# manyeyes/AliParaformerAsr

Hardware: AMD Instinct MI355X
Metric: RTFx (audio-sec/wall-sec), paraformer-large offline, batch 32x30s per GPU, 2 batches in flight per GPU (higher is better)
Workload: dtype f16; 1 GPU; paraformer-large-zh offline, batch 32x30 s synthetic 16 kHz per GPU (BASELINE.json configs[1]), seeded synthetic weights; global_batch=32, samples_per_utt=480000, T_lfr=500, L=167, steps_in_flight=2

## Files before the change

aliparaformerasr_amd/_native.py:

```python
from __future__ import annotations

import ctypes as C
import os

_HERE = os.path.dirname(os.path.abspath(__file__))
LIB_PATH = os.path.join(_HERE, "libparaformer_hip.so")

PF_OK = 0
PF_ERR_INVALID_ARG = -1
PF_ERR_DEVICE = -2
PF_ERR_IO = -3
PF_ERR_FORMAT = -4
PF_ERR_CAPACITY = -5
PF_ERR_UNSUPPORTED = -6
PF_ERR_DISPOSED = -7
PF_ERR_TOKENS = -8
PF_ERR_NULL_SAMPLES = -9
PF_ERR_RECOGNITION = -10

PF_DECODE_SCORES = 1
PF_DECODE_CTC = 2
PF_DECODE_TOPK = 8
PF_DECODE_CTC_BEAM = 16
PF_HOTWORD_STATES_MAX = 4096
# ... 220 lines not shown
    "pf_host_group_sim": (C.c_int, [C.c_int32, C.c_int32, _i32, C.c_int32, C.c_int32, C.c_int32, C.c_int32, C.c_int32, _i64,
                                    C.c_int32, _i32, _i32]),
    "pf_profile_enable": (C.c_int, [_vp, C.c_int32]),
    "pf_profile_reset": (C.c_int, [_vp]),
    "pf_profile_select": (C.c_int, [_vp, C.c_char_p]),
    "pf_profile_get": (C.c_int, [_vp, C.c_char_p, _P(C.c_double), _i64, _P(C.c_double)]),
    "pf_profile_kernel": (C.c_int, [_vp, C.c_char_p, C.c_char_p, C.c_int32]),
    "pf_last_flops": (C.c_int, [_vp, _P(C.c_double)]),
    "pf_op_lfr_cmvn_pad": (C.c_int, [_vp, _P(_f), _i32, C.c_int32, C.c_int32, _f, C.c_int64, _i32]),
    "pf_op_fbank_batch": (C.c_int, [_vp, _P(_f), _i64, C.c_int32, _f, C.c_int64, _i32]),
    "pf_op_qlinear": (C.c_int, [_vp, _f, _f, _f, C.c_int32, C.c_int32, C.c_int32, C.c_int32, C.c_int32, _f, _P(C.c_uint8), _f,
                                _P(C.c_uint8), _f, _i32]),
    "pf_op_argmax": (C.c_int, [_vp, _f, C.c_int64, C.c_int32, _i64]),
    "pf_op_gemm": (C.c_int, [_vp, _f, _f, _f, C.c_int32, C.c_int32, C.c_int32, C.c_int32, _f]),
    "pf_op_gemm_ex": (C.c_int, [_vp, _P(PfGemmDesc), _f, _f, _f]),
    "pf_op_gemm_rc": (C.c_int, [_vp, _P(PfGemmRcDesc), _f, _f, _f, _f, _f]),
    "pf_op_ffn": (C.c_int, [_vp, _f, _f, _f, _f, _f, _f, C.c_int32, C.c_int32, C.c_int32, _f]),
    "pf_op_ffn_fused": (C.c_int, [_vp, _f, _f, _f, _f, _f, _f, _f, _f, C.c_int32, _f, _f]),
    "pf_op_dec_ffn_fused": (C.c_int, [_vp, C.c_void_p, _f, _f, _f]),
    "pf_op_attn_ffn_fused": (C.c_int, [_vp, _vp, _f, _f]),
    "pf_op_fsmn_enc": (C.c_int, [_vp, _f, _f, C.c_int32, C.c_int32, C.c_int32, C.c_int32, _f]),
    "pf_op_linear32": (C.c_int, [_vp, _f, _f, _f, _f, C.c_int32, C.c_int32, C.c_int32, C.c_int32, _f]),
    "pf_op_ffn32": (C.c_int, [_vp, _f, _f, _f, _f, _f, C.c_int32, C.c_int32, C.c_int32, _f]),
    "pf_op_fsmn_dec": (C.c_int, [_vp, _f, _f, _i32, C.c_int32, C.c_int32, C.c_int32, C.c_int32, _f]),
    "pf_op_lstm": (C.c_int, [_vp, _f, _f, C.c_int32, C.c_int32, C.c_int32, C.c_int32, C.c_int32, _f]),
    "pf_op_us_peak": (C.c_int, [_vp, _f, _f, _f, C.c_float, C.c_float, _i32, C.c_float, C.c_int32, C.c_int32, C.c_int32, _f, _f, _f]),
    "pf_op_logsoftmax_argmax": (C.c_int, [_vp, _f, C.c_int64, C.c_int32, _f, _i64]),
    "pf_op_layernorm": (C.c_int, [_vp, _f, _f, _f, C.c_int64, C.c_int32, _f]),
    "pf_op_attention": (C.c_int, [_vp, _f, _f, _f, C.c_int32, C.c_int32, C.c_int32, C.c_int32, _f]),
    "pf_op_fsmn": (C.c_int, [_vp, _f, _f, _f, C.c_int32, C.c_int32, C.c_int32, C.c_int32, _f]),
# ... 115 lines not shown
```

aliparaformerasr_amd/csrc/c_api.cpp:

```cpp
#include <algorithm>
#include <cstring>
#include <deque>
#include <memory>
#include <mutex>

#include "engine.h"
#include "group.h"
#include "online.h"
#include "recognizer.h"
#include "shards_sim.h"

namespace pf {
static thread_local std::string g_last_error;
void set_last_error(const std::string& m) { g_last_error = m; }
}

using namespace pf;

struct pf_engine {
  std::mutex mu;
  std::shared_ptr<Engine> e;
};
struct pf_recognizer {
  std::mutex mu;
// ... 1003 lines not shown
  e->op_qlinear(x, W, bias, M, N, K, relu, x_is_f16, y, xq_out, aparams_out, wq_out, wscale_out, wzp_out);
  return PF_OK;
  PF_CATCH
}
int pf_op_gemm_ex(pf_engine* h, const pf_gemm_desc* d, const float* A, const float* W, float* C) {
  PF_TRY
  std::shared_ptr<Engine> eh_ = E(h);
  Engine* e = eh_.get();
  NEED(d); NEED(A); NEED(W); NEED(C);
  PF_CHECK(d->struct_size == (int32_t)sizeof(pf_gemm_desc), PF_ERR_INVALID_ARG, "pf_gemm_desc.struct_size mismatch");
  std::lock_guard<std::mutex> lk(e->mutex());
  e->op_gemm_ex(*d, A, W, C);
  return PF_OK;
  PF_CATCH
}
int pf_op_gemm_rc(pf_engine* h, const pf_gemm_rc_desc* d, const float* A, const float* W, float* x_out, float* n16_out,
                  float* n32_out) {
  PF_TRY
  std::shared_ptr<Engine> eh_ = E(h);
  Engine* e = eh_.get();
  NEED(d); NEED(A); NEED(W);
  PF_CHECK(d->struct_size == (int32_t)sizeof(pf_gemm_rc_desc), PF_ERR_INVALID_ARG, "pf_gemm_rc_desc.struct_size mismatch");
  PF_CHECK(x_out || n16_out || n32_out, PF_ERR_INVALID_ARG, "gemm_rc: no output requested");
  std::lock_guard<std::mutex> lk(e->mutex());
  e->op_gemm_rc(*d, A, W, x_out, n16_out, n32_out);
  return PF_OK;
  PF_CATCH
}
int pf_op_ffn(pf_engine* h, const float* x, const float* w1, const float* b1, const float* w2, const float* b2,
              const float* resid, int32_t M, int32_t D, int32_t F, float* y) {
// ... 1131 lines not shown
```

aliparaformerasr_amd/csrc/engine.cpp:

```cpp
#include "engine.h"

#include <algorithm>
#include <cmath>
#include <cstdlib>
#include <chrono>
#include <cstring>
#include <set>

#include "hostutil.h"

namespace pf {

static std::mutex g_main_mu;
static std::vector<std::pair<int, hipStream_t>> g_main_streams;
static std::vector<hipStream_t> g_parked;

Engine::Engine(const pf_engine_config& cfg) {
  device_ = cfg.device;
  int ndev = 0;
  hipError_t e = hipGetDeviceCount(&ndev);
  if (e != hipSuccess || ndev <= 0)
    throw Error(PF_ERR_DEVICE, "no HIP device available (this library has no CPU fallback)");
  PF_CHECK(device_ >= 0 && device_ < ndev, PF_ERR_DEVICE, "device ordinal out of range");
  PF_HIP(hipSetDevice(device_));
// ... 12 lines not shown
  fc_.dither_seed = (uint32_t)cfg.dither_seed;
  fc_.window = cfg.window ? cfg.window : "hamming";
  PF_CHECK(fc_.dither >= 0.f && fc_.dither == fc_.dither, PF_ERR_INVALID_ARG, "dither must be >= 0");
  PF_CHECK(fc_.fs == 16000, PF_ERR_UNSUPPORTED, "only fs = 16000 is supported");
  PF_CHECK((cfg.frame_length_ms == 0 || cfg.frame_length_ms == 25) && (cfg.frame_shift_ms == 0 || cfg.frame_shift_ms == 10),
           PF_ERR_UNSUPPORTED, "only frame_length = 25 ms and frame_shift = 10 ms are supported");
  PF_CHECK(cfg.math_mode >= 0 && cfg.math_mode <= 3, PF_ERR_INVALID_ARG,
           "math_mode must be 0 (f16 MFMA), 1 (fp32 MFMA), 2 (dynamic int8 as model.int8.onnx, int8 MFMA) or 3 (exact: split-f16 products)");
  fp32_mode_ = cfg.math_mode == 1 || cfg.math_mode == 3;
  x3_mode_ = cfg.math_mode == 3;
  int8_mode_ = cfg.math_mode == 2;
  { const char* e = getenv("PF_QKV_MIN"); if (e && e[0]) qkv_split_min_tiles_ = atoi(e); }
  { const char* e = getenv("PF_QKV_FILL"); if (e && e[0]) qkv_split_min_fill_ = atoi(e); }
  { const char* e = getenv("PF_FFN_MIN"); if (e && e[0]) ffn_fused_min_rows_ = atoi(e); }
  { const char* e = getenv("PF_DEC_MID"); if (e && e[0]) dec_mid_ = e[0] != '0'; }

  std::vector<float> shift, scale;
  if (cfg.mvn_path && cfg.mvn_path[0]) {
    parse_mvn_text(read_text_file(cfg.mvn_path), shift, scale);
  } else if (cfg.cmvn_shift && cfg.cmvn_scale && cfg.cmvn_dim > 0) {
    shift.assign(cfg.cmvn_shift, cfg.cmvn_shift + cfg.cmvn_dim);
    scale.assign(cfg.cmvn_scale, cfg.cmvn_scale + cfg.cmvn_dim);
  }
  if (!shift.empty()) {
    PF_CHECK(shift.size() == scale.size(), PF_ERR_FORMAT, "am.mvn: shift/scale length mismatch");
    PF_CHECK((int)shift.size() == fc_.lfr_m * fc_.n_mels, PF_ERR_FORMAT, "am.mvn: CMVN dim must equal lfr_m * n_mels");
  }

  uid_ = register_uid();
  try {
// ... 486 lines not shown
    ts_ih_.bias = gb;
    const Tensor& ow = tensor("predictor.out2.weight");
    PF_CHECK(ow.numel == 2 * D, PF_ERR_FORMAT, "weights: predictor.out2.weight shape");
    PF_CHECK(tensor("predictor.out2.bias").numel == 1, PF_ERR_FORMAT, "weights: predictor.out2.bias shape");
    ts_out_w_ = ow.dev;
    ts_out_b_ = tensor("predictor.out2.bias").dev;
    PF_HIP(hipStreamSynchronize(stream_));
    if (fp32_mode_) { ts_up_w32_ = tmp; owned_.push_back(tmp); }
    else PF_HIP(hipFree(tmp));
  }
  dec_ = load_dec_stack("decoder", mc_.dec_layers, mc_.ffn, mc_.kernel, true);
  dec_.out = make_lin("decoder.output", true);
  PF_CHECK(dec_.out.N == mc_.vocab && dec_.out.K == D && dec_.final_w1.K == D && dec_.final_w1.N == mc_.ffn &&
               dec_.final_w2.N == D && dec_.final_w2.K == dec_.final_w1.N,
           PF_ERR_FORMAT, "weights: decoder.final / decoder.output shapes");
  if (mc_.seaco) {
    const Tensor& ew = tensor("seaco.embed.weight");
    PF_CHECK(ew.shape.size() == 2 && ew.shape[1] == D, PF_ERR_FORMAT, "weights: seaco.embed.weight shape");
    seaco_embed_w_ = ew.dev;
    std::vector<float> b1((size_t)4 * D), b2((size_t)4 * D);
    for (int l = 0; l < mc_.seaco_lstm_layers; ++l) {
      const std::string p = "seaco.lstm.l" + std::to_string(l);
      const Tensor& wih = tensor(p + ".weight_ih");
      const Tensor& whh = tensor(p + ".weight_hh");
      const Tensor& bih = tensor(p + ".bias_ih");
      const Tensor& bhh = tensor(p + ".bias_hh");
      PF_CHECK(wih.numel == (int64_t)4 * D * D && whh.numel == (int64_t)4 * D * D && bih.numel == 4 * D && bhh.numel == 4 * D,
               PF_ERR_FORMAT, "weights: seaco.lstm shapes");
      LstmLayer L;
      L.ih.N = 4 * D; L.ih.K = D; L.ih.Kpad = D;
// ... 170 lines not shown
  return true;
}

void Engine::gemm(const char* cls, const Lin& w, const half_t* A, int lda, int M, float* out32, int ld32,
                  half_t* out16, int ld16, const float* resid, int ldr, const float* add2, int ld2, bool relu,
                  int scale_cols, float scale, bool bias, int blocked) {
  GemmArgs g{};
  g.A = A; g.lda = lda; g.W = w.w; g.ldw = w.Kpad; g.bias = bias ? w.bias : nullptr;
  g.M = M; g.N = w.N; g.K = w.Kpad;
  g.out_f32 = out32; g.ldc32 = ld32; g.out_f16 = out16; g.ldc16 = ld16;
  g.resid = resid; g.ldr = ldr; g.add2 = add2; g.ld2 = ld2;
  g.relu = relu ? 1 : 0; g.scale_cols = scale_cols; g.scale = scale;
  g.out_padded = 1;
  g.out_blocked = blocked == 1; g.a_blocked = blocked == 2;
  g.small_ws = small_ws_;
  prof_begin(cls, 2.0 * M * (double)w.N * w.K);
  launch_gemm(stream_, g);
  prof_end(cls);
}

void Engine::gemm_small_call(const char* cls, const Lin& w, GemmSmallArgs g, bool bias) {
  g.W = w.w; g.ldw = w.Kpad; g.bias = bias ? w.bias : nullptr; g.N = w.N; g.K = w.Kpad; g.ws = small_ws_;
  prof_begin(cls, 2.0 * g.M * (double)w.N * w.K);
  launch_gemm_small(stream_, g);
  prof_end(cls);
}

int Engine::num_fbank_frames(int64_t n) const {
  if (fc_.snip_edges) return n < 400 ? 0 : (int)(1 + (n - 400) / 160);
  return (int)((n + 80) / 160);
// ... 1470 lines not shown
```

aliparaformerasr_amd/csrc/engine.h:

```cpp
#pragma once
#include <functional>
#include <map>
#include <mutex>
#include <thread>
#include <string>
#include <vector>

#include "lm.h"
#include "json.h"
#include "kernels.h"
#include "shards.h"

namespace pf {

struct ModelCfg {
  std::string kind = "paraformer";
  int feat_dim = 560, d_model = 512, heads = 4, ffn = 2048, enc_layers = 50, tp_layers = 0, kernel = 11;
  int dec_layers = 16, vocab = 8404;
  float cif_threshold = 1.0f, cif_tail = 0.45f, cif_smooth = 1.0f, cif_noise = 0.0f;
  int cif_l_order = 1, cif_r_order = 1;
  bool cif_cumsum = false;
  bool timestamp_head = false, seaco = false, use_itn = false;
  float cif_smooth2 = 0.25f, cif_noise2 = 0.01f;
  int upsample = 3;
// ... 2 lines not shown
};

struct FrontendCfg {
  int fs = 16000, n_mels = 80, lfr_m = 7, lfr_n = 6;
  bool snip_edges = false;
  float dither = 0.f;
  uint32_t dither_seed = 0;
  std::string window = "hamming";
};

struct Lin {
  half_t* w = nullptr;
  const float* bias = nullptr;
  int N = 0, K = 0, Kpad = 0;
  const float* w32 = nullptr;
};
struct LNp { const float* g = nullptr; const float* b = nullptr; int D = 0; };
struct QLin {
  int8_t* w = nullptr;
  int32_t* colsum = nullptr;
  int32_t* wzp = nullptr;
  float* wscale = nullptr;
  int32_t* dz = nullptr;
  const float* bias = nullptr;
  int N = 0, K = 0, Kpad = 0;
};
struct QAct { int8_t* a = nullptr; int32_t* rowsum = nullptr; float* params = nullptr; };
struct EncLayer {
  LNp norm1, norm2; Lin qkv, out, w1, w2; float* fsmn_wT = nullptr; int d_in = 512;
  half_t* qkv_p = nullptr; float* qkv_bias_p = nullptr;
// ... 131 lines not shown
  void op_vad_segments(const int32_t* levels, const int32_t* T, int B, int ld, int n_mels, const pf_vad_config* cfg, int32_t* seg,
                       int cap, int32_t* n);
  void op_ctc_collapse(const int64_t* ids, const float* scores, const int32_t* lens, int B, int T, int blank, int64_t* ids_out,
                       int32_t* first_out, int32_t* last_out, float* score_out, int cap, int32_t* n_out);
  void online_encoder(const float* speech, int B, int Tc, float* enc_out, float* alphas_out);
  void online_decoder(const float* enc, int B, int Tc, const float* embeds, int L, const int32_t* embeds_len,
                      const float* caches_in, float* logits_out, int64_t* ids_out, float* caches_out);
  int dec_layers() const { return (int)dec_.layers.size(); }

  void op_lfr_cmvn_pad(const float* const* fbank, const int32_t* t80, int B, int sentinel, float* out,
                       int64_t cap, int32_t* tmax);
  void op_fbank_batch(const float* const* samples, const int64_t* n, int B, float* out, int64_t cap, int32_t* t80);
  void op_argmax(const float* x, int64_t rows, int V, int64_t* ids);
  void op_gemm(const float* A, const float* W, const float* bias, int M, int N, int K, int epi, float* C);
  void op_gemm_ex(const pf_gemm_desc& d, const float* A, const float* W, float* C);
  void op_linear32(const float* x, const float* W, const float* bias, const float* resid, int M, int N, int K, bool relu, float* y);
  void op_ffn32(const float* x, const float* W1, const float* b1, const float* W2, const float* b2, int M, int D, int F, float* y);
  void op_gemm_rc(const pf_gemm_rc_desc& d, const float* A, const float* W, float* x_out, float* n16_out, float* n32_out);
  void op_qlinear(const float* x, const float* W, const float* bias, int M, int N, int K, int relu, int x_is_f16, float* y,
                  uint8_t* xq_out, float* aparams_out, uint8_t* wq_out, float* wscale_out, int32_t* wzp_out);
  void op_dec_ffn_fused(const pf_dec_ffn_desc& ds, float* t_out, float* n_out, float* x_out);
  void op_ffn_fused(const float* x, const float* w1, const float* b1, const float* w2, const float* b2, const float* resid,
                    const float* g, const float* be, int M, float* x_out, float* n16_out, const pf_attn_ffn_desc* op = nullptr);
  void op_ffn(const float* x, const float* w1, const float* b1, const float* w2, const float* b2, const float* resid,
              int M, int D, int F, float* y);
  void op_fsmn_enc(const float* v, const float* w, int B, int T, int D, int k, float* y);
  void op_fsmn_dec(const float* tn, const float* w, const int32_t* token_num, int B, int L, int D, int k, float* x);
  void op_lstm(const float* xg, const float* whh, int B, int T3, int D, int ndir, int form, float* hout);
  void op_us_peak(const float* hout, const float* w, const float* b0, float smooth, float noise, const int32_t* token_num, float thr,
                  int B, int T3, int W, float* alphas_raw, float* alphas, float* peak);
// ... 106 lines not shown
  hipStream_t stream_ = nullptr;
  int32_t* plan_host_ = nullptr; int32_t* plan_host_dev_ = nullptr; int plan_host_cap_ = 0;
  void ensure_plan_host(int B);
  void export_plan(int B);
  int32_t read_back_plan(int B);
  hipStream_t aux_stream_ = nullptr;
  hipEvent_t ev_scan_ = nullptr;
  hipStream_t ts_stream_ = nullptr;
  hipEvent_t ev_ts_ = nullptr, ev_enc_ = nullptr;
  bool ts_pending_ = false, ts_defer_copy_ = false;
  size_t ts_copy_floats_ = 0;
  void join_ts();
  void own_hardware_queue_ts();
  void own_hardware_queue();
  bool dec_mid_ = true;
  int ffn_fused_min_rows_ = 1200;
  int qkv_split_min_tiles_ = 256;
  int qkv_split_min_fill_ = 60;
  int cus_ = 256;
  unsigned* lstm_err_ = nullptr;
  void check_async_errors();
  void attention32(const float* q, int64_t q_bs, int q_rs, const float* k, int64_t k_bs, int k_rs, const float* v, int64_t v_bs, int v_rs,
                   float* o, int64_t o_bs, int o_rs, int B, int H, int Lq, int Lk, bool only_operand = false);
  void layernorm32(const float* x, int M, int D, const LNp& ln, float* xn);
  bool x3a_pair_only_ = false;
  bool x3_mode_ = false;
  void x3_forget(const float* W);
  std::map<std::pair<const float*, int>, half_t*> x3w_;
  DevBuf ws_x3a_, ws_x3t_, ws_x3h_;
  bool x3_pair_live_ = false; int x3_pair_M_ = 0, x3_pair_K_ = 0;
// ... 124 lines not shown
```

aliparaformerasr_amd/csrc/engine_ops.cpp:

```cpp
#include "engine.h"

#include <algorithm>
#include <cmath>
#include <cstdlib>
#include <cstring>
#include <limits>
#include <set>

#include "hostutil.h"

namespace pf {

namespace {
constexpr uint32_t kSentinel32 = 0x7FC5A5A5u;
constexpr uint16_t kSentinel16 = 0x7E5Au;
constexpr int kVLead = 64;

inline half_t hostile16(size_t i) {
  const uint16_t bits = (uint16_t)(0x7800u | (uint16_t)((i * 37u) & 0x3FFu) | (uint16_t)((i & 1u) << 15));
  half_t h;
  std::memcpy(&h, &bits, 2);
  return h;
}

// ... 650 lines not shown
    PF_HIP(hipMemcpy2DAsync(C, (size_t)N * 4, base + oC, (size_t)ld32 * 4, (size_t)N * 4, M, hipMemcpyDeviceToHost, stream_));
    PF_HIP(hipStreamSynchronize(stream_));
  } else {
    const size_t rows = ds.out_kind == 2 ? (size_t)round_up(M, 32) : (size_t)M;
    const size_t ld = ds.out_kind == 2 ? (size_t)N : (size_t)ld16;
    std::vector<half_t> tmp(rows * ld);
    PF_HIP(hipMemcpyAsync(tmp.data(), base + oC, tmp.size() * 2, hipMemcpyDeviceToHost, stream_));
    PF_HIP(hipStreamSynchronize(stream_));
    for (int m = 0; m < M; ++m)
      for (int n = 0; n < N; ++n) {
        const size_t idx = ds.out_kind == 2 ? (((size_t)(m >> 5) * (N >> 3) + (n >> 3)) * 32 + (m & 31)) * 8 + (n & 7)
                                            : (size_t)m * ld + n;
        C[(size_t)m * N + n] = (float)tmp[idx];
      }
  }
}

void Engine::op_gemm_rc(const pf_gemm_rc_desc& ds, const float* A, const float* W, float* x_out, float* n16_out,
                        float* n32_out) {
  PF_HIP(hipSetDevice(device_));
  const int M = ds.M, K = ds.K, N = 512;
  PF_CHECK(M > 0 && K > 0 && K % 64 == 0, PF_ERR_INVALID_ARG, "gemm_rc: K must be a positive multiple of 64");
  PF_CHECK(!ds.fsmn_v || (ds.fsmn_w && ds.fsmn_k > 0), PF_ERR_INVALID_ARG, "gemm_rc: FSMN needs weights");
  PF_CHECK((ds.ln_gamma != nullptr) == (ds.ln_beta != nullptr), PF_ERR_INVALID_ARG, "gemm_rc: gamma and beta go together");
  const int64_t Mp = round_up(M, 256) + 128;
  const int k = ds.fsmn_k;
  size_t off = 0;
  const Carve carve{off};
  const size_t o32 = carve((size_t)std::max<int64_t>((int64_t)M * std::max(K, N), (int64_t)N * K) * 4);
  const size_t oA16 = carve((size_t)Mp * K * 2), oW16 = carve((size_t)N * K * 2), ob = carve((size_t)N * 4);
// ... 760 lines not shown
```

aliparaformerasr_amd/csrc/k_gemm.hip:

```cpp
#include "kernels.h"
#include "kdev.h"
#include "exact.h"

#include <cstdlib>
#include <mutex>
#include <type_traits>

namespace pf {
template <int V>
using ic = std::integral_constant<int, V>;

struct GemmDev {
  const half_t* A; const half_t* W; const float* bias;
  float* out_f32; half_t* out_f16; const float* resid; const float* add2;
  int lda, ldw, ldc32, ldc16, ldr, ld2;
  int M, N, K, tiles_m, tiles_n;
  int relu, scale_cols; float scale;
  int out_padded;
  int out_blocked, a_blocked;
  int f16_lo_off;
  int k_wrap, a_wrap, w_wrap;
  float wrap_scale;
  const int32_t* q_rowsum;
  const int32_t* q_colsum;
// ... 648 lines not shown
  d.lda = a.lda; d.ldw = a.ldw; d.ldc32 = a.ldc32; d.ldc16 = a.ldc16; d.ldr = a.ldr; d.ld2 = a.ld2;
  d.M = a.M; d.N = a.N; d.K = a.K;
  d.relu = a.relu; d.scale_cols = a.scale_cols; d.scale = a.scale_cols > 0 ? a.scale : 1.f;
  d.out_padded = a.out_padded;
  d.out_blocked = a.out_blocked; d.a_blocked = a.a_blocked;
  d.f16_lo_off = a.f16_lo_off;
  PF_CHECK(a.f16_lo_off == 0 || (a.out_f16 && !a.out_blocked && a.f16_lo_off % 4 == 0 && a.M > gemm_small_max_rows()),
           PF_ERR_INVALID_ARG, "gemm: the x3 pair output is an option of the fp32-kind epilogue (M above the short-input threshold)");
  d.k_wrap = a.k_wrap; d.a_wrap = a.a_wrap * 2; d.w_wrap = a.w_wrap * 2; d.wrap_scale = a.wrap_scale;
  PF_CHECK(a.k_wrap == 0 || (a.k_wrap > 0 && a.k_wrap < a.K / 64 && a.a_wrap % 64 == 0 && a.w_wrap % 64 == 0 && a.a_wrap <= a.k_wrap * 64 &&
                             a.w_wrap <= a.k_wrap * 64 && !a.a_blocked && !a.out_blocked && a.M > gemm_small_max_rows()),
           PF_ERR_INVALID_ARG, "gemm: K-loop wrap needs 0 < k_wrap < K / 64, cursor steps of whole k-steps inside the range walked so far, row-major operands, M above the short-input threshold");
  PF_CHECK(!a.out_blocked || (a.out_f16 && !a.out_f32 && !a.resid && !a.add2 && a.out_padded && a.N % 64 == 0),
           PF_ERR_INVALID_ARG, "gemm: blocked output needs an f16-only padded result with N % 64 == 0");
  PF_CHECK(!a.a_blocked || a.K % 64 == 0, PF_ERR_INVALID_ARG, "gemm: blocked A operand needs K % 64 == 0");
  if (a.force_mi == 4 || (a.force_mi == 0 && a.small_ws && a.M <= gemm_small_max_rows() && !a.out_blocked && !a.a_blocked)) {
    GemmSmallArgs g{};
    g.A = a.A; g.lda = a.lda; g.W = a.W; g.ldw = a.ldw; g.bias = a.bias; g.M = a.M; g.N = a.N; g.K = a.K;
    g.out_f32 = a.out_f32; g.ldc32 = a.ldc32; g.out_f16 = a.out_f16; g.ldc16 = a.ldc16;
    g.resid = a.resid; g.ldr = a.ldr; g.add2 = a.add2; g.ld2 = a.ld2;
    g.relu = a.relu; g.scale_cols = a.scale_cols; g.scale = a.scale; g.ws = a.small_ws;
    const bool can = !a.out_blocked && !a.a_blocked && gemm_small_applicable(g);
    PF_CHECK(a.force_mi != 4 || can, PF_ERR_INVALID_ARG, "gemm: the short-input kernel does not apply to this problem");
    if (can) { launch_gemm_small(s, g); return; }
  }
  static const float mi_x = [] { const char* e = getenv("PF_GEMM_MI_X"); return e ? (float)atof(e) : 0.6f; }();
  static DeviceOnce once;
  once.run([] {
    set_max_lds((const void*)gemm_f16_pp3<1, 2>, gemm_lds_bytes(2));
    set_max_lds((const void*)gemm_f16_pp3<2, 2>, gemm_lds_bytes(2));
// ... 96 lines not shown
```

aliparaformerasr_amd/csrc/kernels.h:

```cpp
#pragma once
#include "common.h"

namespace pf {

struct GemmArgs {
  const half_t* A; int lda;
  const half_t* W; int ldw;
  const float* bias;
  int M, N, K;
  float* out_f32; int ldc32;
  half_t* out_f16; int ldc16;
  const float* resid; int ldr;
  const float* add2; int ld2;
  int relu;
  int scale_cols; float scale;
  int out_padded;
  int out_blocked;
  int a_blocked;
  float* small_ws;
  int f16_lo_off;
  int k_wrap, a_wrap, w_wrap; float wrap_scale;
  int force_mi;
};
void launch_gemm(hipStream_t s, const GemmArgs& a);
const char* last_gemm_kernel();
void note_gemm_kernel(const char* name);
bool gemm_qkvp_applicable(int M, int K, int lda, int ldw, int ldv);
void launch_qkv_permute(hipStream_t s, const half_t* w, int ldw, const float* bias, half_t* wp, float* bp);
void launch_gemm_qkvp(hipStream_t s, const half_t* A, int lda, const half_t* Wp, int ldw, const float* bias_p, int M, int K,
                      float qscale, half_t* out_qk, half_t* out_v, int ldv);
bool gemm_bigp_applicable(const GemmArgs& a);
void launch_gemm_bigp(hipStream_t s, const GemmArgs& a, int cus);

struct GemmI8Args {
  const int8_t* A; int lda;
  const int8_t* W; int ldw;
  const int32_t* rowsum;
  const int32_t* colsum;
  const int32_t* wzp;
// ... 254 lines not shown
```

aliparaformerasr_amd/engine.py:

```python
from __future__ import annotations

import ctypes as C

import numpy as np

from . import _native as N


def _fp(a: np.ndarray):
    return a.ctypes.data_as(C.POINTER(C.c_float))


def _f32(a) -> np.ndarray:
    return np.ascontiguousarray(a, dtype=np.float32)


class CtcResult:

    def __init__(self, n, ids, first, last, score):
        self.n, self.ids, self.first, self.last, self.score = n, ids, first, last, score

    def tokens(self, b):
        k = int(self.n[b])
        return list(zip(self.ids[b, :k].tolist(), self.first[b, :k].tolist(), self.last[b, :k].tolist(),
# ... 951 lines not shown
                   tile_rows=0, scale_cols=0, scale=1.0) -> np.ndarray:
        A, W = _f32(A), _f32(W)
        M, K = A.shape
        Nn = W.shape[0]
        d = N.PfGemmDesc()
        d.struct_size = C.sizeof(N.PfGemmDesc)
        d.M, d.N, d.K = M, Nn, K
        d.relu, d.out_kind, d.a_blocked, d.tile_rows = int(relu), out_kind, int(a_blocked), tile_rows
        d.scale_cols, d.scale = scale_cols, scale
        keep = [_f32(t) if t is not None else None for t in (bias, resid, add2)]
        d.bias, d.resid, d.add2 = [_fp(t) if t is not None else None for t in keep]
        out = np.zeros((M, Nn), np.float32)
        N.check(self._lib.pf_op_gemm_ex(self._h, C.byref(d), _fp(A), _fp(W), _fp(out)))
        return out

    def op_gemm_rc(self, A, W, bias=None, resid=None, fsmn_v=None, fsmn_w=None, T=0, ln=None, a_blocked=False,
                   want_x=True, want_n16=True, want_n32=True, short_input=False):
        A, W = _f32(A), _f32(W)
        M, K = A.shape
        d = N.PfGemmRcDesc()
        d.struct_size = C.sizeof(N.PfGemmRcDesc)
        d.M, d.K, d.a_blocked, d.T = M, K, int(a_blocked), T
        d.short_input = int(short_input)
        d.split_k = 0
        keep = [_f32(t) if t is not None else None for t in (bias, resid, fsmn_v, fsmn_w)]
        d.bias, d.resid, d.fsmn_v, d.fsmn_w = [_fp(t) if t is not None else None for t in keep]
        d.fsmn_k = keep[3].shape[1] if keep[3] is not None else 0
        g = b = None
        if ln is not None:
            g, b = _f32(ln[0]), _f32(ln[1])
# ... 282 lines not shown
```

include/paraformer_hip.h:

```cpp
#ifndef PARAFORMER_HIP_H_
#define PARAFORMER_HIP_H_

#include <stdint.h>

#ifdef __cplusplus
extern "C" {
#endif

#define PF_ABI_VERSION 6

typedef enum pf_status {
  PF_OK = 0,
  PF_ERR_INVALID_ARG = -1,
  PF_ERR_DEVICE = -2,
  PF_ERR_IO = -3,
  PF_ERR_FORMAT = -4,
  PF_ERR_CAPACITY = -5,
  PF_ERR_UNSUPPORTED = -6,
  PF_ERR_DISPOSED = -7,
  PF_ERR_TOKENS = -8,
  PF_ERR_NULL_SAMPLES = -9,
  PF_ERR_RECOGNITION = -10
} pf_status;

// ... 242 lines not shown
               int32_t M, int32_t N, int32_t K, int32_t epilogue, float* C);
typedef struct pf_gemm_desc {
  int32_t struct_size;
  int32_t M, N, K;
  int32_t relu;
  int32_t out_kind;
  int32_t a_blocked;
  int32_t tile_rows;
  int32_t scale_cols;
  float scale;
  const float* bias;
  const float* resid;
  const float* add2;
} pf_gemm_desc;
int pf_op_gemm_ex(pf_engine* e, const pf_gemm_desc* d, const float* A, const float* W, float* C);
typedef struct pf_gemm_rc_desc {
  int32_t struct_size;
  int32_t M, K;
  int32_t a_blocked;
  int32_t T;
  int32_t fsmn_k;
  const float* bias;
  const float* resid;
  const float* fsmn_v;
  const float* fsmn_w;
  const float* ln_gamma;
  const float* ln_beta;
  int32_t short_input;
  int32_t split_k;
} pf_gemm_rc_desc;
// ... 176 lines not shown
```

Before: 113,300 audio-sec/wall-sec.

## Add panel-resident GEMM kernel for decoder KV and output projections

Adds a new GEMM kernel that keeps a 128-row panel of the activation A (K=512) resident in LDS. Each workgroup streams pre-retiled weight blocks from a register prefetch ring, overlapping the epilogue stores of one block with the MFMA work of the next. The decoder kv_all and vocabulary output weights are retiled once at load time into a panel image. The kernel is selected by default for eligible GEMMs with M above 512. It costs extra device memory for the retiled weights and adds a complex kernel with its own store and sharing heuristics.

Result: faster. 115,300 audio-sec/wall-sec, median of 6 (+1.7%).

```diff
diff --git a/aliparaformerasr_amd/_native.py b/aliparaformerasr_amd/_native.py
--- a/aliparaformerasr_amd/_native.py
+++ b/aliparaformerasr_amd/_native.py
@@ -258,6 +258,7 @@
     "pf_op_argmax": (C.c_int, [_vp, _f, C.c_int64, C.c_int32, _i64]),
     "pf_op_gemm": (C.c_int, [_vp, _f, _f, _f, C.c_int32, C.c_int32, C.c_int32, C.c_int32, _f]),
     "pf_op_gemm_ex": (C.c_int, [_vp, _P(PfGemmDesc), _f, _f, _f]),
+    "pf_op_gemm_panel": (C.c_int, [_vp, C.c_int32, C.c_int32, C.c_int32, C.c_int32, C.c_int32, _f, _f, _f, _f]),
     "pf_op_gemm_rc": (C.c_int, [_vp, _P(PfGemmRcDesc), _f, _f, _f, _f, _f]),
     "pf_op_ffn": (C.c_int, [_vp, _f, _f, _f, _f, _f, _f, C.c_int32, C.c_int32, C.c_int32, _f]),
     "pf_op_ffn_fused": (C.c_int, [_vp, _f, _f, _f, _f, _f, _f, _f, _f, C.c_int32, _f, _f]),
diff --git a/aliparaformerasr_amd/csrc/c_api.cpp b/aliparaformerasr_amd/csrc/c_api.cpp
--- a/aliparaformerasr_amd/csrc/c_api.cpp
+++ b/aliparaformerasr_amd/csrc/c_api.cpp
@@ -1041,6 +1041,17 @@
   return PF_OK;
   PF_CATCH
 }
+int pf_op_gemm_panel(pf_engine* h, int32_t M, int32_t N, int32_t out_kind, int32_t form, int32_t padded, const float* bias, const float* A,
+                     const float* W, float* C) {
+  PF_TRY
+  std::shared_ptr<Engine> eh_ = E(h);
+  Engine* e = eh_.get();
+  NEED(A); NEED(W); NEED(C);
+  std::lock_guard<std::mutex> lk(e->mutex());
+  e->op_gemm_panel(M, N, out_kind, form, padded, bias, A, W, C);
+  return PF_OK;
+  PF_CATCH
+}
 int pf_op_gemm_rc(pf_engine* h, const pf_gemm_rc_desc* d, const float* A, const float* W, float* x_out, float* n16_out,
                   float* n32_out) {
   PF_TRY
diff --git a/aliparaformerasr_amd/csrc/engine.cpp b/aliparaformerasr_amd/csrc/engine.cpp
--- a/aliparaformerasr_amd/csrc/engine.cpp
+++ b/aliparaformerasr_amd/csrc/engine.cpp
@@ -50,6 +50,7 @@
   { const char* e = getenv("PF_QKV_FILL"); if (e && e[0]) qkv_split_min_fill_ = atoi(e); }
   { const char* e = getenv("PF_FFN_MIN"); if (e && e[0]) ffn_fused_min_rows_ = atoi(e); }
   { const char* e = getenv("PF_DEC_MID"); if (e && e[0]) dec_mid_ = e[0] != '0'; }
+  { const char* e = getenv("PF_GEMM_PANEL"); if (e && e[0]) gemm_panel_ = e[0] != '0'; }
 
   std::vector<float> shift, scale;
   if (cfg.mvn_path && cfg.mvn_path[0]) {
@@ -566,6 +567,12 @@
   PF_CHECK(dec_.out.N == mc_.vocab && dec_.out.K == D && dec_.final_w1.K == D && dec_.final_w1.N == mc_.ffn &&
                dec_.final_w2.N == D && dec_.final_w2.K == dec_.final_w1.N,
            PF_ERR_FORMAT, "weights: decoder.final / decoder.output shapes");
+  if (gemm_panel_ && !fp32_mode_ && !int8_mode_)
+    for (Lin* l : {&dec_.kv_all, &dec_.out})
+      if (l->w && l->N > 0 && l->K == 512 && l->Kpad == 512) {
+        l->w_panel = (half_t*)dalloc(gemm_panel_image_bytes(l->N));
+        launch_gemm_panel_retile(stream_, l->w, l->Kpad, l->N, l->w_panel);
+      }
   if (mc_.seaco) {
     const Tensor& ew = tensor("seaco.embed.weight");
     PF_CHECK(ew.shape.size() == 2 && ew.shape[1] == D, PF_ERR_FORMAT, "weights: seaco.embed.weight shape");
@@ -766,6 +773,7 @@
   g.out_padded = 1;
   g.out_blocked = blocked == 1; g.a_blocked = blocked == 2;
   g.small_ws = small_ws_;
+  g.W_panel = gemm_panel_ ? w.w_panel : nullptr;
   prof_begin(cls, 2.0 * M * (double)w.N * w.K);
   launch_gemm(stream_, g);
   prof_end(cls);
diff --git a/aliparaformerasr_amd/csrc/engine.h b/aliparaformerasr_amd/csrc/engine.h
--- a/aliparaformerasr_amd/csrc/engine.h
+++ b/aliparaformerasr_amd/csrc/engine.h
@@ -40,6 +40,7 @@
   const float* bias = nullptr;
   int N = 0, K = 0, Kpad = 0;
   const float* w32 = nullptr;
+  half_t* w_panel = nullptr;
 };
 struct LNp { const float* g = nullptr; const float* b = nullptr; int D = 0; };
 struct QLin {
@@ -201,6 +202,7 @@
   void op_argmax(const float* x, int64_t rows, int V, int64_t* ids);
   void op_gemm(const float* A, const float* W, const float* bias, int M, int N, int K, int epi, float* C);
   void op_gemm_ex(const pf_gemm_desc& d, const float* A, const float* W, float* C);
+  void op_gemm_panel(int M, int N, int out_kind, int form, int padded, const float* bias, const float* A, const float* W, float* C);
   void op_linear32(const float* x, const float* W, const float* bias, const float* resid, int M, int N, int K, bool relu, float* y);
   void op_ffn32(const float* x, const float* W1, const float* b1, const float* W2, const float* b2, int M, int D, int F, float* y);
   void op_gemm_rc(const pf_gemm_rc_desc& d, const float* A, const float* W, float* x_out, float* n16_out, float* n32_out);
@@ -337,6 +339,7 @@
   void own_hardware_queue_ts();
   void own_hardware_queue();
   bool dec_mid_ = true;
+  bool gemm_panel_ = true;
   int ffn_fused_min_rows_ = 1200;
   int qkv_split_min_tiles_ = 256;
   int qkv_split_min_fill_ = 60;
diff --git a/aliparaformerasr_amd/csrc/engine_ops.cpp b/aliparaformerasr_amd/csrc/engine_ops.cpp
--- a/aliparaformerasr_amd/csrc/engine_ops.cpp
+++ b/aliparaformerasr_amd/csrc/engine_ops.cpp
@@ -688,6 +688,71 @@
         C[(size_t)m * N + n] = (float)tmp[idx];
       }
   }
+}
+
+void Engine::op_gemm_panel(int M, int N, int out_kind, int form, int padded, const float* bias, const float* A, const float* W, float* C) {
+  PF_HIP(hipSetDevice(device_));
+  constexpr int K = 512;
+  PF_CHECK(M > 0 && N > 0, PF_ERR_INVALID_ARG, "gemm_panel: empty problem");
+  PF_CHECK(out_kind == 0 || out_kind == 1, PF_ERR_INVALID_ARG, "gemm_panel: out_kind must be 0 (fp32) or 1 (f16)");
+  PF_CHECK(form == 0 || form == 1 || form == 2 || form == 7, PF_ERR_INVALID_ARG, "gemm_panel: form must be 0, 1, 2 or 7");
+  const int64_t Mp = round_up(M, 256) + 128, Np = round_up(N, 256);
+  const int ld = out_kind == 1 ? N + 64 : (int)round_up(N, 4);
+  PF_CHECK(ld % 4 == 0, PF_ERR_INVALID_ARG, "gemm_panel: the f16 form needs N % 4 == 0");
+  const size_t esz = out_kind == 1 ? 2 : 4;
+  size_t off = 0;
+  const Carve carve{off};
+  const size_t oA = carve((size_t)M * K * 4), oW = carve((size_t)N * K * 4), ob = carve((size_t)N * 4);
+  const size_t oA16 = carve((size_t)Mp * K * 2), oW16 = carve((size_t)Np * K * 2), oI = carve(gemm_panel_image_bytes(N));
+  const size_t oC = carve((size_t)Mp * ld * esz);
+  ensure(ws_tmp_, off);
+  char* base = (char*)ws_tmp_.p;
+  PF_HIP(hipMemsetD16Async((hipDeviceptr_t)(base + oA16), 0x7E00, (size_t)Mp * K, stream_));
+  PF_HIP(hipMemsetD16Async((hipDeviceptr_t)(base + oW16), 0x7E00, (size_t)Np * K, stream_));
+  PF_HIP(hipMemcpyAsync(base + oA, A, (size_t)M * K * 4, hipMemcpyHostToDevice, stream_));
+  launch_f32_to_f16(stream_, (const float*)(base + oA), M, K, K, (half_t*)(base + oA16), K);
+  PF_HIP(hipMemcpyAsync(base + oW, W, (size_t)N * K * 4, hipMemcpyHostToDevice, stream_));
+  launch_f32_to_f16(stream_, (const float*)(base + oW), N, K, K, (half_t*)(base + oW16), K);
+  launch_gemm_panel_retile(stream_, (const half_t*)(base + oW16), K, N, (half_t*)(base + oI));
+  if (bias) PF_HIP(hipMemcpyAsync(base + ob, bias, (size_t)N * 4, hipMemcpyHostToDevice, stream_));
+  if (out_kind == 0) fill_sentinel32(stream_, base + oC, (size_t)Mp * ld);
+  else fill_sentinel16(stream_, base + oC, (size_t)Mp * ld);
+  GemmArgs g{};
+  g.A = (half_t*)(base + oA16); g.lda = K; g.W = (half_t*)(base + oW16); g.ldw = K; g.W_panel = (half_t*)(base + oI);
+  g.bias = bias ? (const float*)(base + ob) : nullptr;
+  g.M = M; g.N = N; g.K = K;
+  g.out_padded = padded ? 1 : 0;
+  g.force_mi = form;
+  if (out_kind == 0) { g.out_f32 = (float*)(base + oC); g.ldc32 = ld; }
+  else { g.out_f16 = (half_t*)(base + oC); g.ldc16 = ld; }
+  static const int reps = [] { const char* e = getenv("PF_OP_REPEAT"); return e ? std::max(1, atoi(e)) : 1; }();
+  for (int r = 0; r < reps; ++r) {
+    prof_begin(r == 0 ? "gemm_op" : "gemm_op_warm", 2.0 * M * (double)N * K);
+    launch_gemm(stream_, g);
+    prof_end(r == 0 ? "gemm_op" : "gemm_op_warm");
+  }
+  std::vector<char> h((size_t)Mp * ld * esz);
+  PF_HIP(hipMemcpyAsync(h.data(), base + oC, h.size(), hipMemcpyDeviceToHost, stream_));
+  PF_HIP(hipStreamSynchronize(stream_));
+  const int64_t guard = padded ? round_up(M, 256) : M;
+  for (int64_t m = 0; m < Mp; ++m)
+    for (int n = 0; n < ld; ++n) {
+      const size_t i = (size_t)m * ld + n;
+      const bool is_sent = out_kind == 1 ? reinterpret_cast<const uint16_t*>(h.data())[i] == kSentinel16
+                                         : reinterpret_cast<const uint32_t*>(h.data())[i] == kSentinel32;
+      const char* why = nullptr;
+      if (m < M && n < N) { if (is_sent) why = "was not written"; }
+      else if (n >= N) { if (!is_sent) why = "was written: a column beyond N"; }
+      else if (m >= guard && !is_sent) why = "was written: a row the destination does not declare writable";
+      if (why)
+        throw Error(PF_ERR_DEVICE, "gemm_panel (" + std::to_string(M) + " x " + std::to_string(N) + ", ld " + std::to_string(ld) + "): cell (" +
+                                       std::to_string(m) + ", " + std::to_string(n) + ") " + why);
+    }
+  for (int m = 0; m < M; ++m)
+    for (int n = 0; n < N; ++n) {
+      const size_t i = (size_t)m * ld + n;
+      C[(size_t)m * N + n] = out_kind == 1 ? (float)reinterpret_cast<const half_t*>(h.data())[i] : reinterpret_cast<const float*>(h.data())[i];
+    }
 }
 
 void Engine::op_gemm_rc(const pf_gemm_rc_desc& ds, const float* A, const float* W, float* x_out, float* n16_out,
diff --git a/aliparaformerasr_amd/csrc/k_gemm.hip b/aliparaformerasr_amd/csrc/k_gemm.hip
--- a/aliparaformerasr_amd/csrc/k_gemm.hip
+++ b/aliparaformerasr_amd/csrc/k_gemm.hip
@@ -686,6 +686,15 @@
   PF_CHECK(!a.out_blocked || (a.out_f16 && !a.out_f32 && !a.resid && !a.add2 && a.out_padded && a.N % 64 == 0),
            PF_ERR_INVALID_ARG, "gemm: blocked output needs an f16-only padded result with N % 64 == 0");
   PF_CHECK(!a.a_blocked || a.K % 64 == 0, PF_ERR_INVALID_ARG, "gemm: blocked A operand needs K % 64 == 0");
+  {
+    const bool can = gemm_panel_applicable(a);
+    PF_CHECK(a.force_mi != 7 || can, PF_ERR_INVALID_ARG, "gemm: the panel-resident kernel does not apply to this problem");
+    const int min_rows = std::max(gemm_panel_min_rows(), a.small_ws ? gemm_small_max_rows() : 0);
+    if (can && (a.force_mi == 7 || (a.force_mi == 0 && a.M > min_rows))) {
+      launch_gemm_panel(s, a, device_cus());
+      return;
+    }
+  }
   if (a.force_mi == 4 || (a.force_mi == 0 && a.small_ws && a.M <= gemm_small_max_rows() && !a.out_blocked && !a.a_blocked)) {
     GemmSmallArgs g{};
     g.A = a.A; g.lda = a.lda; g.W = a.W; g.ldw = a.ldw; g.bias = a.bias; g.M = a.M; g.N = a.N; g.K = a.K;
diff --git a/aliparaformerasr_amd/csrc/k_gemm_panel.hip b/aliparaformerasr_amd/csrc/k_gemm_panel.hip
--- /dev/null
+++ b/aliparaformerasr_amd/csrc/k_gemm_panel.hip
@@ -0,0 +1,350 @@
+#include "kernels.h"
+#include "kdev.h"
+
+#include <algorithm>
+#include <cstdlib>
+#include <type_traits>
+
+namespace pf {
+
+struct PanelDev {
+  const half_t* A; const half_t* Wp; const float* bias;
+  float* out_f32; half_t* out_f16;
+  int lda, ldc32, ldc16;
+  int M, N, nblk, S;
+  int bias_first;
+  int al16;
+};
+
+constexpr int GP_ROWS = 128, GP_PANEL = GP_ROWS * 512 * 2, GP_KB = GP_ROWS * 128, GP_SCR = 2048;
+constexpr int GP_LDS = GP_PANEL + 8 * GP_SCR;
+constexpr int GP_BLK_BYTES = 64 * 512 * 2;
+constexpr int GP_LINE = 1152;
+
+template <int ST>
+__device__ __forceinline__ void gp_st16(void* p, h8 v) {
+  if constexpr (ST == 2) asm volatile("global_store_dwordx4 %0, %1, off sc1" ::"v"(p), "v"(v) : "memory");
+  else *reinterpret_cast<h8*>(p) = v;
+}
+template <int ST>
+__device__ __forceinline__ void gp_st16(void* p, float4 v) {
+  if constexpr (ST == 2) {
+    const f4v x = {v.x, v.y, v.z, v.w};
+    asm volatile("global_store_dwordx4 %0, %1, off sc1" ::"v"(p), "v"(x) : "memory");
+  } else *reinterpret_cast<float4*>(p) = v;
+}
+
+template <int KIND, int PF, int XD, int ST>
+__global__ __launch_bounds__(512, 1) void gemm_panel_kernel(PanelDev p) {
+  static_assert(64 % PF == 0 && 32 % (XD + 1) == 0, "the rings run on across blocks");
+  constexpr int XR = XD + 1;
+  extern __shared__ __attribute__((aligned(16))) char smem[];
+  const int tid = threadIdx.x, lane = tid & 63;
+  const int wave = __builtin_amdgcn_readfirstlane(tid >> 6);
+  const int lh = lane >> 5, l31 = lane & 31;
+  const int rh = wave >> 2, cg = wave & 3;
+  const int bid = blockIdx.x;
+  const int panel = bid / p.S, share = bid - panel * p.S;
+  const int m0 = panel * GP_ROWS;
+  const int b0 = (int)((long long)share * p.nblk / p.S), nb = (int)((long long)(share + 1) * p.nblk / p.S) - b0;
+  const int rot = (((bid >> 3) & 3) * nb) >> 2;
+  const int steps = nb > cg ? (nb - cg + 3) >> 2 : 0;
+  auto blk_of = [&](int st) __attribute__((always_inline)) -> int {
+    const int q = cg + 4 * st + rot;
+    return b0 + (q >= nb ? q - nb : q);
+  };
+  auto swz = [](int row) __attribute__((always_inline)) -> int { return (row >> 1) & 7; };
+
+  const unsigned lane16 = (unsigned)lane * 16u;
+  auto wbase = [&](int blk) __attribute__((always_inline)) -> const char* {
+    return reinterpret_cast<const char*>(p.Wp) + (size_t)blk * GP_BLK_BYTES;
+  };
+  auto wld = [&](const char* base, int pos) __attribute__((always_inline)) -> h8 {
+    return *reinterpret_cast<const h8*>(base + pos * 1024 + lane16);
+  };
+  auto bias_ld = [&](int blk) __attribute__((always_inline)) -> float {
+    int n = blk * 64 + lane;
+    n = n < p.N ? n : p.N - 1;
+    return p.bias ? p.bias[n] : 0.f;
+  };
+  char* const scr = smem + GP_PANEL + wave * GP_SCR;
+  const char* cur = wbase(steps ? blk_of(0) : b0);
+  h8 ring[PF];
+  float bnx = 0.f;
+  if (steps) {
+#pragma unroll
+    for (int i = 0; i < PF; ++i) ring[i] = wld(cur, i);
+    bnx = bias_ld(blk_of(0));
+  }
+
+  {
+    const int srow = lane >> 3, schunk = lane & 7;
+#pragma unroll
+    for (int h = 0; h < 2; ++h) {
+      const int row = (wave * 2 + h) * 8 + srow;
+      int m = m0 + row;
+      m = m < p.M ? m : p.M - 1;
+      const char* src = reinterpret_cast<const char*>(p.A + (size_t)m * p.lda) + ((schunk ^ swz(row)) << 4);
+#pragma unroll
+      for (int kb = 0; kb < 8; ++kb) glds16(src + kb * 128, smem + kb * GP_KB + (wave * 2 + h) * 1024);
+    }
+  }
+  wait_vmcnt<0>();
+  reinterpret_cast<float*>(scr + GP_LINE)[lane] = bnx;
+  wait_lgkm0();
+  __builtin_amdgcn_s_barrier();
+  if (steps == 0) return;
+
+  unsigned xo[2][4];
+#pragma unroll
+  for (int i = 0; i < 2; ++i)
+#pragma unroll
+    for (int ss = 0; ss < 4; ++ss) {
+      const int ra = rh * 64 + i * 32 + l31;
+      xo[i][ss] = (unsigned)(ra * 128 + (((2 * ss + lh) ^ swz(ra)) << 4));
+    }
+  auto xld = [&](int s, int i) __attribute__((always_inline)) -> h8 {
+    return *reinterpret_cast<const h8*>(smem + (s >> 2) * GP_KB + xo[i][s & 3]);
+  };
+  h8 xf[XR][2];
+#pragma unroll
+  for (int s0 = 0; s0 < XD; ++s0)
+#pragma unroll
+    for (int i = 0; i < 2; ++i) xf[s0][i] = xld(s0, i);
+
+  f16x acc[2][2];
+  const int mrow = m0 + rh * 64;
+  int pn0 = 0;
+  h4 hq[2][2][4];
+  f16x pq[2][2];
+  const float* pl = reinterpret_cast<const float*>(scr + GP_LINE);
+
+  char* const wp16 = scr + (lane & 7) * 144 + lh * 8;
+  const char* const rp16 = scr + (lane >> 3) * 144 + (lane & 7) * 16;
+  h8 rowv;
+  auto pass_write = [&](auto IC, int q) __attribute__((always_inline)) {
+    constexpr int i = decltype(IC)::value;
+    if ((l31 >> 3) == q) {
+#pragma unroll
+      for (int j = 0; j < 2; ++j)
+#pragma unroll
+        for (int g = 0; g < 4; ++g) *reinterpret_cast<h4a*>(wp16 + (j * 32 + 8 * g) * 2) = hq[i][j][g];
+    }
+  };
+  auto pass_read = [&]() __attribute__((always_inline)) {
+    asm volatile("" ::: "memory");
+    rowv = *reinterpret_cast<const h8a*>(rp16);
+    asm volatile("" ::: "memory");
+  };
+  auto pass_store = [&](int idx) __attribute__((always_inline)) {
+    const int m = mrow + idx * 8 + (lane >> 3), n = pn0 + (lane & 7) * 8;
+    if (m >= p.M) return;
+    half_t* o = p.out_f16 + (size_t)m * p.ldc16 + n;
+    if (p.al16 && n + 8 <= p.N) gp_st16<ST>(o, rowv);
+    else if (n + 8 <= p.N) {
+      *reinterpret_cast<h4*>(o) = h4{rowv[0], rowv[1], rowv[2], rowv[3]};
+      *reinterpret_cast<h4*>(o + 4) = h4{rowv[4], rowv[5], rowv[6], rowv[7]};
+    } else {
+#pragma unroll
+      for (int e = 0; e < 8; ++e)
+        if (n + e < p.N) o[e] = rowv[e];
+    }
+  };
+  char* const wp32 = scr + (l31 & 3) * 272 + lh * 16;
+  const char* const rp32 = scr + (lane >> 4) * 272 + (lane & 15) * 16;
+  float4 segv;
+  auto chunk_write = [&](auto IC, int c8) __attribute__((always_inline)) {
+    constexpr int i = decltype(IC)::value;
+    if ((l31 >> 2) == c8) {
+#pragma unroll
+      for (int j = 0; j < 2; ++j)
+#pragma unroll
+        for (int g = 0; g < 4; ++g)
+          *reinterpret_cast<float4a*>(wp32 + (j * 32 + 8 * g) * 4) =
+              make_float4(pq[i][j][4 * g + 0], pq[i][j][4 * g + 1], pq[i][j][4 * g + 2], pq[i][j][4 * g + 3]);
+    }
+  };
+  auto chunk_read = [&]() __attribute__((always_inline)) {
+    asm volatile("" ::: "memory");
+    segv = *reinterpret_cast<const float4a*>(rp32);
+    asm volatile("" ::: "memory");
+  };
+  auto chunk_store = [&](int c) __attribute__((always_inline)) {
+    const int m = mrow + c * 4 + (lane >> 4), n = pn0 + (lane & 15) * 4;
+    if (m >= p.M) return;
+    float4 v = segv;
+    const float4 pb4 = *reinterpret_cast<const float4a*>(pl + (lane & 15) * 4);
+    v.x = fmaxf(v.x + pb4.x, -INFINITY); v.y = fmaxf(v.y + pb4.y, -INFINITY);
+    v.z = fmaxf(v.z + pb4.z, -INFINITY); v.w = fmaxf(v.w + pb4.w, -INFINITY);
+    float* o = p.out_f32 + (size_t)m * p.ldc32 + n;
+    if (n + 4 <= p.N) gp_st16<ST>(o, v);
+    else {
+      if (n < p.N) o[0] = v.x;
+      if (n + 1 < p.N) o[1] = v.y;
+      if (n + 2 < p.N) o[2] = v.z;
+    }
+  };
+  auto drain = [&](int s) __attribute__((always_inline)) {
+    if constexpr (KIND == 1) {
+      const int idx = s >> 2;
+      if ((s & 3) == 0) { if (idx < 4) pass_write(std::integral_constant<int, 0>{}, idx & 3); else pass_write(std::integral_constant<int, 1>{}, idx & 3); }
+      if ((s & 3) == 1) pass_read();
+      if ((s & 3) == 2) pass_store(idx);
+    } else {
+      const int c = s >> 1;
+      if ((s & 1) == 0) { if (c < 8) chunk_write(std::integral_constant<int, 0>{}, c & 7); else chunk_write(std::integral_constant<int, 1>{}, c & 7); }
+      else { chunk_read(); chunk_store(c); }
+    }
+  };
+
+  for (int st = 0; st < steps; ++st) {
+    const int blk = blk_of(st);
+    const bool last = st + 1 == steps;
+    const int blk_n = last ? blk : blk_of(st + 1);
+    const char* nxt = wbase(blk_n);
+    const int n0 = blk * 64;
+    const bool bf = KIND == 1 && p.bias_first && n0 + 64 <= p.N;
+    const float* bl = reinterpret_cast<const float*>(scr + GP_LINE + (st & 1) * 256);
+    asm volatile("" ::: "memory");
+#pragma unroll
+    for (int j = 0; j < 2; ++j)
+#pragma unroll
+      for (int g = 0; g < 4; ++g) {
+        float4 b4 = make_float4(0.f, 0.f, 0.f, 0.f);
+        if (bf) b4 = *reinterpret_cast<const float4a*>(bl + j * 32 + 8 * g + 4 * lh);
+#pragma unroll
+        for (int i = 0; i < 2; ++i) {
+          acc[i][j][4 * g + 0] = b4.x; acc[i][j][4 * g + 1] = b4.y; acc[i][j][4 * g + 2] = b4.z; acc[i][j][4 * g + 3] = b4.w;
+        }
+      }
+    bnx = bias_ld(blk_n);
+#pragma unroll
+    for (int s = 0; s < 32; ++s) {
+#pragma unroll
+      for (int i = 0; i < 2; ++i) xf[(s + XD) % XR][i] = xld((s + XD) & 31, i);
+      h8 wf[2];
+#pragma unroll
+      for (int j = 0; j < 2; ++j) {
+        const int pos = 2 * s + j;
+        wf[j] = ring[pos % PF];
+        ring[pos % PF] = pos + PF < 64 ? wld(cur, pos + PF) : wld(nxt, pos + PF - 64);
+      }
+      if (st > 0) drain(s);
+      if (s == 31) {
+        reinterpret_cast<float*>(scr + GP_LINE + ((st + 1) & 1) * 256)[lane] = bnx;
+        asm volatile("" ::: "memory");
+      }
+#pragma unroll
+      for (int i = 0; i < 2; ++i)
+#pragma unroll
+        for (int j = 0; j < 2; ++j) acc[i][j] = __builtin_amdgcn_mfma_f32_32x32x16_f16(wf[j], xf[s % XR][i], acc[i][j], 0, 0, 0);
+      __builtin_amdgcn_sched_barrier(0);
+    }
+    asm volatile("" ::: "memory");
+    if constexpr (KIND == 1) {
+#pragma unroll
+      for (int j = 0; j < 2; ++j)
+#pragma unroll
+        for (int g = 0; g < 4; ++g) {
+          float4 b4 = make_float4(0.f, 0.f, 0.f, 0.f);
+          if (!bf) b4 = *reinterpret_cast<const float4a*>(bl + j * 32 + 8 * g + 4 * lh);
+#pragma unroll
+          for (int i = 0; i < 2; ++i) {
+            float v0 = acc[i][j][4 * g + 0], v1 = acc[i][j][4 * g + 1], v2 = acc[i][j][4 * g + 2], v3 = acc[i][j][4 * g + 3];
+            if (!bf) { v0 += b4.x; v1 += b4.y; v2 += b4.z; v3 += b4.w; }
+            hq[i][j][g] = h4{(half_t)fmaxf(v0, -INFINITY), (half_t)fmaxf(v1, -INFINITY), (half_t)fmaxf(v2, -INFINITY),
+                             (half_t)fmaxf(v3, -INFINITY)};
+          }
+        }
+    } else {
+#pragma unroll
+      for (int i = 0; i < 2; ++i)
+#pragma unroll
+        for (int j = 0; j < 2; ++j) pq[i][j] = acc[i][j];
+      pl = bl;
+    }
+    pn0 = n0;
+    cur = nxt;
+  }
+#pragma unroll
+  for (int s = 0; s < 32; ++s) drain(s);
+}
+
+__global__ void gemm_panel_retile_kernel(const half_t* __restrict__ W, int ldw, int N, int nblk, half_t* __restrict__ img) {
+  const int64_t pc = (int64_t)blockIdx.x * blockDim.x + threadIdx.x;
+  if (pc >= (int64_t)nblk * 4096) return;
+  const int l = (int)(pc & 63), j = (int)(pc >> 6) & 1, t = (int)(pc >> 7) & 31, b = (int)(pc >> 12);
+  const int row = b * 64 + j * 32 + (l & 31);
+  h8 v;
+#pragma unroll
+  for (int e = 0; e < 8; ++e) v[e] = (_Float16)0.f;
+  if (row < N) {
+    const half_t* src = W + (size_t)row * ldw + 16 * t + 8 * (l >> 5);
+#pragma unroll
+    for (int e = 0; e < 8; ++e) v[e] = src[e];
+  }
+  *reinterpret_cast<h8*>(img + (size_t)pc * 8) = v;
+}
+
+size_t gemm_panel_image_bytes(int N) { return (size_t)cdiv(N, 64) * GP_BLK_BYTES; }
+void launch_gemm_panel_retile(hipStream_t s, const half_t* W, int ldw, int N, half_t* img) {
+  const int nblk = cdiv(N, 64);
+  if (nblk == 0) return;
+  hipLaunchKernelGGL(gemm_panel_retile_kernel, dim3(nblk * 16), dim3(256), 0, s, W, ldw, N, nblk, img);
+  PF_HIP(hipGetLastError());
+}
+
+int gemm_panel_min_rows() {
+  static const int v = [] { const char* e = getenv("PF_PANEL_M"); return e && e[0] ? atoi(e) : 512; }();
+  return v;
+}
+
+bool gemm_panel_applicable(const GemmArgs& a) {
+  return a.K == 512 && a.W_panel && a.M > 0 && a.N > 0 && ((a.out_f16 != nullptr) != (a.out_f32 != nullptr)) && !a.resid && !a.add2 &&
+         !a.relu && a.scale_cols == 0 && !a.out_blocked && !a.a_blocked && a.f16_lo_off == 0 && a.k_wrap == 0 && a.lda % 8 == 0 &&
+         (a.out_f16 ? a.ldc16 % 4 == 0 : a.ldc32 % 4 == 0);
+}
+
+int gemm_panel_shares(int panels, int N, int cus) {
+  static const int forced = [] { const char* e = getenv("PF_PANEL_S"); return e && e[0] ? atoi(e) : 0; }();
+  const int cap = std::max(1, N / 512);
+  if (forced > 0) return std::min(forced, std::max(1, cdiv(N, 64)));
+  int S = 1;
+  while (S < cap && (double)panels * S < 0.9 * cus) ++S;
+  return S;
+}
+
+void launch_gemm_panel(hipStream_t s, const GemmArgs& a, int cus) {
+  PF_CHECK(gemm_panel_applicable(a), PF_ERR_INVALID_ARG, "gemm: the panel-resident kernel does not apply to this problem");
+  PanelDev d{};
+  d.A = a.A; d.Wp = a.W_panel; d.bias = a.bias; d.out_f32 = a.out_f32; d.out_f16 = a.out_f16;
+  d.lda = a.lda; d.ldc32 = a.ldc32; d.ldc16 = a.ldc16;
+  d.M = a.M; d.N = a.N; d.nblk = cdiv(a.N, 64);
+  const int panels = cdiv(a.M, GP_ROWS);
+  d.S = gemm_panel_shares(panels, a.N, cus);
+  d.bias_first = a.out_f16 && a.out_padded && (a.ldc16 & 7) == 0;
+  d.al16 = a.out_f16 && (a.ldc16 & 7) == 0 && (reinterpret_cast<uintptr_t>(a.out_f16) & 15) == 0;
+  static const int st = [] { const char* e = getenv("PF_PANEL_ST"); return e && e[0] ? atoi(e) : -1; }();
+  static DeviceOnce once;
+  once.run([] {
+    set_max_lds((const void*)gemm_panel_kernel<1, 16, 1, 2>, GP_LDS);
+    set_max_lds((const void*)gemm_panel_kernel<1, 16, 1, 0>, GP_LDS);
+    set_max_lds((const void*)gemm_panel_kernel<2, 8, 1, 2>, GP_LDS);
+    set_max_lds((const void*)gemm_panel_kernel<2, 8, 1, 0>, GP_LDS);
+  });
+  const dim3 grid(panels * d.S), block(512);
+  if (a.out_f16) {
+    const bool sc1 = st < 0 ? true : st == 2;
+    note_gemm_kernel(sc1 ? "gemm_panel_kernel<1, 16, 1, 2>" : "gemm_panel_kernel<1, 16, 1, 0>");
+    if (sc1) hipLaunchKernelGGL((gemm_panel_kernel<1, 16, 1, 2>), grid, block, GP_LDS, s, d);
+    else hipLaunchKernelGGL((gemm_panel_kernel<1, 16, 1, 0>), grid, block, GP_LDS, s, d);
+  } else {
+    const bool sc1 = st < 0 ? false : st == 2;
+    note_gemm_kernel(sc1 ? "gemm_panel_kernel<2, 8, 1, 2>" : "gemm_panel_kernel<2, 8, 1, 0>");
+    if (sc1) hipLaunchKernelGGL((gemm_panel_kernel<2, 8, 1, 2>), grid, block, GP_LDS, s, d);
+    else hipLaunchKernelGGL((gemm_panel_kernel<2, 8, 1, 0>), grid, block, GP_LDS, s, d);
+  }
+  PF_HIP(hipGetLastError());
+}
+
+}
diff --git a/aliparaformerasr_amd/csrc/kernels.h b/aliparaformerasr_amd/csrc/kernels.h
--- a/aliparaformerasr_amd/csrc/kernels.h
+++ b/aliparaformerasr_amd/csrc/kernels.h
@@ -21,8 +21,15 @@
   int f16_lo_off;
   int k_wrap, a_wrap, w_wrap; float wrap_scale;
   int force_mi;
+  const half_t* W_panel;
 };
 void launch_gemm(hipStream_t s, const GemmArgs& a);
+size_t gemm_panel_image_bytes(int N);
+void launch_gemm_panel_retile(hipStream_t s, const half_t* W, int ldw, int N, half_t* img);
+bool gemm_panel_applicable(const GemmArgs& a);
+int gemm_panel_min_rows();
+int gemm_panel_shares(int panels, int N, int cus);
+void launch_gemm_panel(hipStream_t s, const GemmArgs& a, int cus);
 const char* last_gemm_kernel();
 void note_gemm_kernel(const char* name);
 bool gemm_qkvp_applicable(int M, int K, int lda, int ldw, int ldv);
diff --git a/aliparaformerasr_amd/engine.py b/aliparaformerasr_amd/engine.py
--- a/aliparaformerasr_amd/engine.py
+++ b/aliparaformerasr_amd/engine.py
@@ -989,6 +989,17 @@
         N.check(self._lib.pf_op_gemm_ex(self._h, C.byref(d), _fp(A), _fp(W), _fp(out)))
         return out
 
+    def op_gemm_panel(self, A, W, bias=None, f16_out=False, form=7, padded=False) -> np.ndarray:
+        A, W = _f32(A), _f32(W)
+        M, K = A.shape
+        Nn = W.shape[0]
+        assert K == 512 and W.shape[1] == 512
+        b = _f32(bias) if bias is not None else None
+        out = np.zeros((M, Nn), np.float32)
+        N.check(self._lib.pf_op_gemm_panel(self._h, M, Nn, int(f16_out), form, int(padded), _fp(b) if b is not None else None,
+                                           _fp(A), _fp(W), _fp(out)))
+        return out
+
     def op_gemm_rc(self, A, W, bias=None, resid=None, fsmn_v=None, fsmn_w=None, T=0, ln=None, a_blocked=False,
                    want_x=True, want_n16=True, want_n32=True, short_input=False):
         A, W = _f32(A), _f32(W)
diff --git a/include/paraformer_hip.h b/include/paraformer_hip.h
--- a/include/paraformer_hip.h
+++ b/include/paraformer_hip.h
@@ -280,6 +280,8 @@
   const float* add2;
 } pf_gemm_desc;
 int pf_op_gemm_ex(pf_engine* e, const pf_gemm_desc* d, const float* A, const float* W, float* C);
+int pf_op_gemm_panel(pf_engine* e, int32_t M, int32_t N, int32_t out_kind, int32_t form, int32_t padded, const float* bias,
+                     const float* A, const float* W, float* C);
 typedef struct pf_gemm_rc_desc {
   int32_t struct_size;
   int32_t M, K;
```
